# hydradarpa/kalman-hydra

Measured on AMD Instinct MI355X. Metric: frames/sec (Brox flow + EKF update) at 1024^2, higher is better.
Workload: dtype f32 (flow, renders) / f64 (EKF sums and state)

## Files before the change

kalman-hydra_amd/csrc/chol_flow_kernels.h:

```cpp
#pragma once
#include <hip/hip_runtime.h>
#include "dense_kernels.h"

#define FLOW_NT 256
#ifdef HM_STAMP
#define HM_CHAIN_STAMP(c, k) do { if (g_stamp && (threadIdx.x & 63) == 0) g_stamp[(size_t)(4096 + (c)) * 8 + (k)] = clock64(); } while (0)
#else
#define HM_CHAIN_STAMP(c, k) do { } while (0)
#endif
#define FLOW_SENTINEL 0x7FF8DEADBEEF0001ull
#define FLOW_POLL_LIMIT 4000000

struct FlowArgs {
    const double *A;
    double *L;
    double *Lt;
    double *Tinv;
    double *P;
    int n, nrows, nb, nbr;
    unsigned *ctl;
    int stall;
};

__device__ __forceinline__ unsigned long long flow_ld_bits(const double *p)
// ... 346 lines not shown
    double acc = 0.0;
    for (int j = threadIdx.x; j < n; j += 256) {
        const double h = H[(size_t)row * n + j];
        A[(size_t)row * n + j] = invW0[(size_t)row * n + j] + h;
        acc += h * (X0[j] + -1.0 * X[j]);
    }
    for (int o = 32; o > 0; o >>= 1) acc += __shfl_down(acc, o, 64);
    if ((threadIdx.x & 63) == 0) s[threadIdx.x >> 6] = acc;
    __syncthreads();
    if (threadIdx.x == 0) A[(size_t)rhs_row * n + row] = Hz[row] - (((s[0] + s[1]) + s[2]) + s[3]);
}

struct PrepArgs {
    const double *out;
    int N, vsplit, esplit;
    double eZ, eJ, eM, d;
    const int *nb_off, *nb_u, *nb_e;
    const double *invW0, *X0, *X;
    double *A, *Hz, *Hzc;
    int n, rhs_row;
    FlowArgs f;
};

__device__ __forceinline__ double d_job_sum(const double *__restrict__ out, int job, int parts, int idx)
{
    const double *src = out + (size_t)job * MEAS_VSPLIT_MAX * MEAS_OUT;
    double v = src[idx];
    for (int q = 1; q < parts; q++) v += src[q * MEAS_OUT + idx];
    return v;
}

#define PREP_MAX_ENTRIES (4 * (EKF_MAX_STAR + 2))
__global__ __launch_bounds__(256) void k_solve_prep(PrepArgs p)
{
    __shared__ double s_term[PREP_MAX_ENTRIES];
    __shared__ double s_hz;
    const int row = blockIdx.x, t = threadIdx.x, n = p.n;
    if (row >= (int)gridDim.x - FLOW_FILL_WGS) {
        flow_fill_blocks(p.f, (row - ((int)gridDim.x - FLOW_FILL_WGS)) * 256 + t, 256 * FLOW_FILL_WGS);
        return;
    }
    flow_fill_row(p.f, row, t, 256);
    if (row >= n) {
        if (row != p.rhs_row)
            for (int j = t; j < n; j += 256) p.A[(size_t)row * n + j] = 0.0;
        return;
    }
    double *Arow = p.A + (size_t)row * n;
    const double *Wrow = p.invW0 + (size_t)row * n;
    {
        double w[4];
#pragma unroll
        for (int q = 0; q < 4; q++) w[q] = (t + 256 * q < n) ? Wrow[t + 256 * q] : 0.0;
#pragma unroll
        for (int q = 0; q < 4; q++)
            if (t + 256 * q < n) Arow[t + 256 * q] = w[q];
        for (int j = t + 1024; j < n; j += 256) Arow[j] = Wrow[j];
    }
    const int N = p.N, n2 = 2 * N;
    const int v = (row % n2) >> 1, ca = (row & 1) + (row >= n2 ? 2 : 0);
    const int deg = p.nb_off[v + 1] - p.nb_off[v];
    const int entries = min(PREP_MAX_ENTRIES, 4 * (deg + 1));
    double val = 0.0;
    int col = 0;
    if (t < entries) {
        const int q = t >> 2, cb = t & 3;
        int idx = -1, job, parts, u;
        bool weighted;
        if (q == 0) {
            u = v; job = v; parts = p.vsplit;
            const int lo = min(ca, cb), hi = max(ca, cb);
            const int tab[4][4] = {{A_XX, A_XY, A_XVX, A_XVY}, {-1, A_YY, A_YVX, A_YVY}, {-1, -1, A_VXVX, -1}, {-1, -1, -1, A_VYVY}};
            idx = tab[lo][hi];
            weighted = hi < 2;
        } else {
            u = p.nb_u[p.nb_off[v] + q - 1];
            job = N + p.nb_e[p.nb_off[v] + q - 1]; parts = p.esplit;
            const int c1 = v < u ? ca : cb, c2 = v < u ? cb : ca;
            const int tab[4][4] = {{B_XX, B_XY, B_XVX, B_XVY}, {B_YX, B_YY, B_YVX, B_YVY}, {B_VXX, B_VXY, B_VXVX, -1},
                                   {B_VYX, B_VYY, -1, B_VYVY}};
            idx = tab[c1][c2];
            weighted = c1 < 2 && c2 < 2;
        }
        col = 2 * u + (cb & 1) + (cb >= 2 ? n2 : 0);
        if (idx >= 0) {
            const double raw = d_job_sum(p.out, job, parts, idx);
            val = (weighted ? raw : raw / p.eJ) / p.d / p.d;
        }
        s_term[t] = val * (p.X0[col] + -1.0 * p.X[col]);
    } else if (t == 255) {
        double c[4] = {0.0, 0.0, 0.0, 0.0};
        if (ca < 2) {
            const int b0 = ca == 0 ? A_X : A_Y;
            c[0] = d_job_sum(p.out, v, p.vsplit, b0) / p.eZ; c[1] = d_job_sum(p.out, v, p.vsplit, b0 + 1) / p.eJ;
            c[2] = -d_job_sum(p.out, v, p.vsplit, b0 + 2) / p.eJ; c[3] = d_job_sum(p.out, v, p.vsplit, b0 + 3) / p.eM;
        } else if (ca == 2) {
            c[1] = d_job_sum(p.out, v, p.vsplit, A_VX) / p.eJ;
        } else {
            c[2] = -d_job_sum(p.out, v, p.vsplit, A_VY) / p.eJ;
        }
        const double hz = (((c[0] + c[1]) + c[2]) + c[3]) / p.d / 2;
        p.Hz[row] = hz;
        for (int ch = 0; ch < 4; ch++) p.Hzc[(size_t)row * 4 + ch] = c[ch] / p.d / 2;
        s_hz = hz;
    }
    __syncthreads();
    if (t < entries) Arow[col] = Wrow[col] + val;
    if (t == 0) {
        double acc = 0.0;
        for (int i = 0; i < entries; i++) acc += s_term[i];
        p.A[(size_t)p.rhs_row * n + row] = s_hz - acc;
    }
}
```

kalman-hydra_amd/csrc/ekf.hip:

```cpp
#include "hm_common.h"
#include "ekf_kernels.h"
#include "dense_kernels.h"
#include "chol_flow_kernels.h"
#include "project_kernels.h"
#include "predict_kernels.h"
#include "view_kernels.h"
#include "body_kernels.h"
#include "roi_kernels.h"
#include "smooth_kernels.h"
#include <algorithm>
#include <atomic>
#include <chrono>
#include <cmath>
#include <condition_variable>
#include <cstring>
#include <functional>
#include <mutex>
#include <set>
#include <thread>
#include <utility>
#include <vector>

struct Helper {
    std::thread th;
// ... 38 lines not shown
    }
    void stop()
    {
        {
            std::unique_lock<std::mutex> lk(m);
            cv.wait(lk, [&] { return !busy; });
            quit = true;
            cv.notify_all();
        }
        if (th.joinable()) th.join();
    }
};

struct hm_ctx {
    int device, W, H, N, T, E, njobs;
    HmOwner own{1};
    Helper helper;
    bool helper_used = false;
    int tail_async = 1;
    double eps_Z, eps_J, eps_M;
    hipStream_t stream;
    int *d_tri, *d_star_off, *d_star_tri, *d_edges;
    int *d_nb_off = nullptr, *d_nb_u = nullptr, *d_nb_e = nullptr;
    float *d_uv;
    uint8_t *d_tex;
    std::vector<int> edges;
    uint8_t *d_yim, *d_ym;
    float *d_yfx, *d_yfy, *d_yfxm, *d_yfym;
    bool obs_owned = true;
    const uint8_t *o_yim, *o_ym;
    const float *o_yfx, *o_yfy;
    bool have_tex, have_obs, have_ref;
    Targets ref, P, Q;
    TriSetup *d_setup, *d_cfgs;
    int4 *d_ubox;
    int *d_tlist = nullptr, *d_tcount = nullptr;
    unsigned *d_tmask = nullptr;
    double *d_X, *d_out, *d_partial;
    uint8_t *d_im8, *d_m8;
    std::vector<double> X0;
    double *d_HTH;
    double *d_H, *d_Hz, *d_Hzc, *d_invW0, *d_Af[2], *d_T[2], *d_step, *d_Wtmp, *d_X0, *d_Xn, *d_Wprior, *d_gain, *d_Awork, *d_Lt[2];
    std::vector<double> upd_X0;
    int upd_last = -1, upd_prev = -1;
    double *d_Wres;
    double *pin;
// ... 322 lines not shown
    step(upload(h->own, &h->d_star_off, off.data(), off.size()));
    step(upload(h->own, &h->d_star_tri, flat.data(), flat.size()));
    step(upload(h->own, &h->d_edges, h->edges.data(), h->edges.size()));
    {
        std::vector<std::vector<std::pair<int, int>>> nb(N);
        for (int e = 0; e < h->E; e++) {
            const int a = h->edges[2 * e], b = h->edges[2 * e + 1];
            nb[a].push_back(std::make_pair(b, e));
            nb[b].push_back(std::make_pair(a, e));
        }
        std::vector<int> noff(N + 1, 0), nu, ne;
        for (int v = 0; v < N; v++) {
            std::sort(nb[v].begin(), nb[v].end());
            noff[v + 1] = noff[v] + (int)nb[v].size();
            for (const auto &q : nb[v]) { nu.push_back(q.first); ne.push_back(q.second); }
            if (rc == HM_OK && 4 * ((int)nb[v].size() + 1) > PREP_MAX_ENTRIES) {
                hm_set_error("hm_ctx_create: vertex %d has %d neighbours, limit %d", v, (int)nb[v].size(), PREP_MAX_ENTRIES / 4 - 1);
                rc = HM_ERR_ARG;
            }
        }
        step(upload(h->own, &h->d_nb_off, noff.data(), noff.size()));
        step(upload(h->own, &h->d_nb_u, nu.data(), nu.size()));
        step(upload(h->own, &h->d_nb_e, ne.data(), ne.size()));
    }
    hipError_t e = hipSuccess;
    auto dev = [&](auto **p, size_t bytes) { if (e == hipSuccess) e = h->own.alloc(p, bytes); };
    if (rc == HM_OK) {
        const char *pe = getenv("HYDRA_MI_EKF_PRIORITY");
        e = h->own.stream(&h->stream, !(pe && atoi(pe) == 0));
        dev(&h->d_tex, n);
        dev(&h->d_yim, n);
        dev(&h->d_ym, n);
        dev(&h->d_yfx, n * sizeof(float));
        dev(&h->d_yfy, n * sizeof(float));
        dev(&h->d_yfxm, n * sizeof(float));
        dev(&h->d_yfym, n * sizeof(float));
        dev(&h->d_setup, (size_t)T * sizeof(TriSetup));
        dev(&h->d_cfgs, (size_t)N * MEAS_NCFG * (EKF_MAX_STAR + 1) * sizeof(TriSetup));
        dev(&h->d_ubox, (size_t)N * UBOX_STRIDE * sizeof(int4));
        dev(&h->d_tmask, (size_t)N * TMASK_STRIDE * sizeof(unsigned));
        dev(&h->d_tlist, (size_t)N * TMASK_STRIDE * sizeof(int));
        dev(&h->d_tcount, (size_t)N * sizeof(int));
        dev(&h->d_X, (size_t)4 * N * sizeof(double));
        dev(&h->d_out, (size_t)h->njobs * MEAS_VSPLIT_MAX * MEAS_OUT * sizeof(double));
        dev(&h->d_partial, (size_t)h->red_blocks * 4 * sizeof(double));
        h->ntiles = hm_cdiv(W, RI_W) * hm_cdiv(H, 8);
        dev(&h->d_tpart, (size_t)h->ntiles * RI_NV * sizeof(double));
        dev(&h->d_im8, n);
        dev(&h->d_m8, n);
        const size_t n4 = (size_t)4 * N, nn = n4 * n4 * sizeof(double);
        dev(&h->d_H, nn);
        dev(&h->d_HTH, nn);
        if (e == hipSuccess) e = hipMemsetAsync(h->d_HTH, 0, nn, h->stream);
        dev(&h->d_invW0, nn);
        const size_t nn_aug = (size_t)(hm_cdiv((int)n4, DNB) * DNB + DNB) * n4 * sizeof(double);
        dev(&h->d_Af[0], nn_aug);
        dev(&h->d_Af[1], nn_aug);
        dev(&h->d_Awork, nn_aug);
        const size_t ld_bytes = (size_t)hm_cdiv((int)n4, DNB) * DNB * DNB * sizeof(double);
        dev(&h->d_T[0], nn);
        dev(&h->d_T[1], nn);
        dev(&h->d_step, n4 * sizeof(double));
        dev(&h->d_Lt[0], ld_bytes);
        dev(&h->d_Lt[1], ld_bytes);
        dev(&h->d_Wtmp, nn);
        dev(&h->d_flowP, 3 * ld_bytes);
        dev(&h->d_flowctl, 4 * sizeof(unsigned));
        if (e == hipSuccess) e = hipMemsetAsync(h->d_flowctl, 0, 4 * sizeof(unsigned), h->stream);
        dev(&h->d_Hz, n4 * sizeof(double));
        dev(&h->d_Hzc, n4 * 4 * sizeof(double));
        dev(&h->d_Wprior, nn);
        dev(&h->d_gain, n4 * 3 * sizeof(double));
        h->pin_n = 2 * (n4 + RES_HEAD + n4 * 4 + n4 * 3) + 2;
        if (e == hipSuccess) e = h->own.host_alloc(&h->pin, h->pin_n * sizeof(double), hipHostMallocCoherent);
        if (e == hipSuccess) memset(h->pin, 0, h->pin_n * sizeof(double));
        h->pin_scratch = (int *)(h->pin + h->pin_n - 2);
        h->resv.assign(n4 + RES_HEAD, 0.0);
        h->tailv.assign(n4 * 7, 0.0);
        dev(&h->d_X0, n4 * sizeof(double));
        dev(&h->pool.hdr, (size_t)4 * N * sizeof(int));
        dev(&h->pool.overflow, sizeof(int));
        dev(&h->d_area, (size_t)N * sizeof(int));
        h->pool.area = h->d_area;
        if (e == hipSuccess) e = pool_alloc(h, (long long)8 * W * H);
        dev(&h->d_Xn, n4 * sizeof(double));
        for (Targets *t : {&h->ref, &h->P, &h->Q})
            if (e == hipSuccess) e = alloc_targets(h->own, *t, n);
    }
    if (e != hipSuccess) {
        hm_set_error("hm_ctx_create: device allocation failed: %s", hipGetErrorString(e));
        step(HM_ERR_HIP);
// ... 33 lines not shown
        HM_ARG(value >= 2 && value <= 2048, "hm_ctx_tune: chol_flow_wgs must be in 2..2048 (the chain workgroup and at least one task workgroup)");
        h->flow_wgs = value;
    } else if (!strcmp(key, "render_rows")) {
        HM_ARG(value == 8 || value == 16, "hm_ctx_tune: render_rows must be 8 or 16");
        h->render_rows = value;
    } else if (!strcmp(key, "chol_flow_stall")) {
        HM_ARG(value >= 0 && value <= 100000, "hm_ctx_tune: chol_flow_stall must be in 0..100000");
        h->flow_stall = value;
    } else if (!strcmp(key, "result_delay")) {
        HM_ARG(value >= 0 && value <= 5000, "hm_ctx_tune: result_delay must be in 0..5000 (microseconds)");
        h->result_delay = value;
    } else if (!strcmp(key, "tail_async")) {
        HM_ARG(value == 0 || value == 1, "hm_ctx_tune: tail_async must be 0 or 1");
        h->tail_async = value;
    } else if (!strcmp(key, "tail_split")) {
        HM_ARG(value == 0 || value == 1, "hm_ctx_tune: tail_split must be 0 or 1");
        h->tail_split = value;
    } else if (!strcmp(key, "newton_fail")) {
        HM_ARG(value == 0 || value == 1, "hm_ctx_tune: newton_fail must be 0 or 1");
        h->newton_fail = value;
    } else if (!strcmp(key, "speculate")) {
        HM_ARG(value == 0 || value == 1, "hm_ctx_tune: speculate must be 0 or 1");
        h->speculate = value;
    } else if (!strcmp(key, "edge_split")) {
        HM_ARG(value >= 1 && value <= MEAS_VSPLIT_MAX, "hm_ctx_tune: edge_split must be in 1..%d", MEAS_VSPLIT_MAX);
        h->esplit = value;
    } else if (!strcmp(key, "body_stats_cap")) {
        HM_ARG(value >= 1 && value <= BODY_STATS_CAP, "hm_ctx_tune: body_stats_cap must be in 1..%d", BODY_STATS_CAP);
        h->stats_cap = value;
    } else if (!strcmp(key, "body_rec_chunk")) {
        HM_ARG(value >= 0, "hm_ctx_tune: body_rec_chunk must be >= 0 (0: the default size)");
        h->rec_chunk = value;
    } else {
        hm_set_error("hm_ctx_tune: unknown key '%s'", key);
        return HM_ERR_ARG;
    }
    return HM_OK;
}
extern "C" void *hm_ctx_stream(hm_ctx_t h)
{
    (void)ctx_join(h);
    return h ? (void *)h->stream : nullptr;
}
extern "C" int hm_ctx_sync(hm_ctx_t h)
{
    HM_ARG(h != nullptr, "hm_ctx_sync: NULL handle");
// ... 394 lines not shown

extern "C" int hm_error(hm_ctx_t h, const double *X, int masked, double err[4], float *fx, float *fy)
{
    HM_ARG(h && X && err, "hm_error: NULL argument");
    HM_JOIN(h);
    NEED_TEX(h, "hm_error");
    NEED_OBS(h, "hm_error");
    HM_HIP(hipSetDevice(h->device));
    HM_HIP(hipMemcpyAsync(h->d_X, X, (size_t)4 * h->N * sizeof(double), hipMemcpyHostToDevice, h->stream));
    int rc = render_iter(h, h->d_X, h->P, true, masked, false, 2.0);
    if (rc) return rc;
    const int n = h->W * h->H;
    if (fx) HM_HIP(hipMemcpyAsync(fx, h->P.fx, (size_t)n * sizeof(float), hipMemcpyDeviceToHost, h->stream));
    if (fy) HM_HIP(hipMemcpyAsync(fy, h->P.fy, (size_t)n * sizeof(float), hipMemcpyDeviceToHost, h->stream));
    HM_HIP(hipMemcpyAsync(h->h_tpart.data(), h->d_tpart, (size_t)render_strips(h) * RI_NV * sizeof(double), hipMemcpyDeviceToHost, h->stream));
    HM_HIP(stream_wait(h->stream));
    double s6[RI_NV];
    hm_tile_partial_sums(h->h_tpart.data(), render_strips(h), s6);
    for (int k = 0; k < 4; k++) err[k] = s6[k];
    return HM_OK;
}

static int measure_dev(hm_ctx *h, const double *dX, bool ref_ready, double deltaX, int masked, bool regions_ready = false,
                       bool scatter = true)
{
    if (!ref_ready) {
        int rc = render_iter(h, dX, h->ref, false, masked, !regions_ready, deltaX);
        if (rc) return rc;
        regions_ready = true;
    }
    MeasureArgs a;
    measure_args(h, dX, deltaX, masked, a);
    if (!regions_ready) hipLaunchKernelGGL(k_star_regions, dim3(h->N), dim3(REGION_NT), 0, h->stream, a, h->d_area);
    hipLaunchKernelGGL(k_measure_vertex, dim3(h->N, h->vsplit), dim3(MEAS_NT), 0, h->stream, a,
                       (const TriSetup *)h->d_cfgs, (const int4 *)h->d_ubox, (const unsigned *)h->d_tmask);
    if (h->E > 0) hipLaunchKernelGGL(k_measure_edge, dim3(h->E, h->esplit), dim3(MEAS_NT), 0, h->stream, a);
    if (scatter) {
        ScatterArgs s = {h->d_out, h->d_edges, h->N, h->E, h->vsplit, h->esplit, h->eps_Z, h->eps_J, h->eps_M, deltaX, h->d_HTH, h->d_Hz, h->d_Hzc};
        hipLaunchKernelGGL(k_hth_scatter, dim3(hm_cdiv(h->njobs, 4)), dim3(256), 0, h->stream, s);
    }
    HM_HIP(hipGetLastError());
    return HM_OK;
}

static void measure_args(hm_ctx *h, const double *dX, double deltaX, int masked, MeasureArgs &a)
{
    a.m = Mesh{h->W, h->H, h->N, h->T, h->d_tri, h->d_uv, h->d_tex};
    a.topo = StarTopo{h->d_star_off, h->d_star_tri, h->d_edges, h->E};
    a.ref = h->ref;
    a.obs = obs_of(h, masked);
    a.X = dX;
    a.delta = deltaX;
    a.out = h->d_out;
    a.pool = h->pool;
    a.vsplit = h->vsplit;
    a.esplit = h->esplit;
    a.iZ = 1.0 / h->eps_Z; a.iJ = 1.0 / h->eps_J; a.iM = 1.0 / h->eps_M;
    a.cfgs = h->d_cfgs;
    a.ubox = h->d_ubox;
// ... 57 lines not shown
    if (!first_done) hipLaunchKernelGGL(k_chol_first, dim3(1), dim3(64), 0, st, A, Lt, n);
    for (int k = 0; k < nb; k++) {
        const int mr = nbr - k - 1, mc = std::max(nb - k - 1, 1);
        hipLaunchKernelGGL(k_chol_step, dim3((mc + k + 1) * (mr + 1)), dim3(256), 0, st, A, L, Lt, T, M, n, nrows, nb, k, mc, mc + k + 1, mr + 1);
    }
}

static void chol_inverse(hm_ctx *h, int n, const double *T, double *out, hipStream_t st = nullptr)
{
    const int nb = hm_cdiv(n, DNB);
    hipLaunchKernelGGL(k_ttt, dim3(nb, nb), dim3(256), 0, st ? st : h->stream, T, n, out);
}

static int flow_status(hm_ctx *h, const char *who)
{
    if (!h->chol_flow) return HM_OK;
    unsigned ctl[2] = {0, 0};
    HM_HIP(hipMemcpyAsync(ctl, h->d_flowctl, sizeof ctl, hipMemcpyDeviceToHost, h->stream));
    HM_HIP(hipStreamSynchronize(h->stream));
    if (ctl[1]) { hm_set_error("%s: the factorisation launch gave up waiting for a block (chol_flow time-out)", who); return HM_ERR_HIP; }
    return HM_OK;
}

static double *solve_step(hm_ctx *h, int slot, double deltaX)
{
    const int n4 = 4 * h->N;
    double *A = h->d_Awork;
    const int rhs_index = hm_cdiv(n4, DNB) * DNB;
    double *rhs_row = A + (size_t)rhs_index * n4;
    {
        const int nb = hm_cdiv(n4, DNB), nrows = aug_rows(n4);
        PrepArgs p;
        p.out = h->d_out; p.N = h->N; p.vsplit = h->vsplit; p.esplit = h->esplit;
        p.eZ = h->eps_Z; p.eJ = h->eps_J; p.eM = h->eps_M; p.d = deltaX;
        p.nb_off = h->d_nb_off; p.nb_u = h->d_nb_u; p.nb_e = h->d_nb_e;
        p.invW0 = h->d_invW0; p.X0 = h->d_X0; p.X = h->d_X;
        p.A = A; p.Hz = h->d_Hz; p.Hzc = h->d_Hzc; p.n = n4; p.rhs_row = rhs_index;
        p.f = FlowArgs{A, h->d_Af[slot], h->d_Lt[slot], h->d_T[slot], h->d_flowP, n4, nrows, nb, hm_cdiv(nrows, DNB), h->d_flowctl, 0};
        hipLaunchKernelGGL(k_solve_prep, dim3(nrows + FLOW_FILL_WGS), dim3(256), 0, h->stream, p);
    }
    if (h->d_Wres == h->d_Wtmp) h->d_Wres = nullptr;
    chol_factor(h, A, h->d_Af[slot], h->d_Lt[slot], h->d_T[slot], h->d_Wtmp, n4, true, h->chol_flow != 0);
    const double *yrow = h->d_Af[slot] + (rhs_row - A);
    hipLaunchKernelGGL(k_tvec, dim3(hm_cdiv(n4, TV_COLS)), dim3(TV_COLS * TV_ROWS), 0, h->stream, h->d_T[slot], n4, yrow, h->d_step, h->d_X0,
                       h->d_Xn);
    return h->d_step;
}

static int prior_inverse(hm_ctx *h, const double *W_prior, hipStream_t st = nullptr)
{
    if (!st) st = h->stream;
    const int n4 = 4 * h->N;
    const size_t nnb = (size_t)n4 * n4 * sizeof(double);
    if (W_prior)
        HM_HIP(hipMemcpyAsync(h->d_Wprior, W_prior, nnb, hipMemcpyHostToDevice, st));
    else if (h->d_Wres != h->d_Wprior)
        HM_HIP(hipMemcpyAsync(h->d_Wprior, h->d_Wres, nnb, hipMemcpyDeviceToDevice, st));
    if (!h->chol_flow) HM_HIP(hipMemcpyAsync(h->d_Awork, h->d_Wprior, nnb, hipMemcpyDeviceToDevice, st));
    h->d_Wres = h->d_Wprior;
    HM_HIP(hipMemsetAsync(h->d_flowctl, 0, 4 * sizeof(unsigned), st));
    chol_factor(h, h->chol_flow ? h->d_Wprior : h->d_Awork, h->d_Af[0], h->d_Lt[0], h->d_Wtmp, h->d_invW0, n4, false, false, st);
    chol_inverse(h, n4, h->d_Wtmp, h->d_invW0, st);
// ... 318 lines not shown
    auto chain_collect = [&]() -> int {
        int r = hb_wait(h->stream3, h->pin_n4 + n4, 0, (size_t)n4 + 2, hb_stamp(h->n4_ticket), h->n4v.data(), "hm_update_run (state prediction)");
        h->n4_pending = false;
        if (r) return r;
        r = hb_wait(h->stream3, h->pin_pm + n4, 0, (size_t)n4 + 1, hb_stamp(h->pm_ticket), h->pmv.data(), "hm_update_run (projectmask)");
        if (r) return r;
        h->chain_pred.assign(h->n4v.begin(), h->n4v.begin() + n4);
        h->chain_proj.assign(h->pmv.begin(), h->pmv.begin() + n4);
        h->chain_its = (int)h->n4v[n4];
        h->chain_moved = (int)h->pmv[n4];
        if (h->n4v[n4 + 1] != 0.0) return 2;
        X0 = h->chain_proj; Xcur = X0; Xold = X0;
        h->upd_X0 = X0;
        h->X0 = X0;
        return HM_OK;
    };
    bool collected = !chained;
    if (!chained) HM_HIP(hipMemcpyAsync(h->d_X, h->d_X0, (size_t)n4 * sizeof(double), hipMemcpyDeviceToDevice, h->stream));
    double *const pin_res = h->pin, *const pin_tail = h->pin + 2 * ((size_t)n4 + RES_HEAD);
    const double *const res = h->resv.data();
    int niter = 0, accepted = 0;
    bool reverted = false, conv = false, ref_ready = false, regions_ahead = false, grown = false;
    double eold = 0.0;
    bool spec = false;
    auto unspec = [&]() {
        if (spec) { std::swap(h->ref, h->P); std::swap(h->d_X, h->d_Xn); spec = false; }
    };
    for (int it = 0; it < max_iter; it++) {
        if (!spec) {
            rc = measure_dev(h, h->d_X, ref_ready, deltaX, masked, regions_ahead, false);
            if (rc) return rc;
        }
        spec = false;
        if (next_mask && it == 0) {
            HM_HIP(h->own.event(&h->ev_m0));
            HM_HIP(hipEventRecord(h->ev_m0, h->stream));
        }
        if (collected) h->X0 = Xcur;
        h->have_ref = true;
        const int slot = h->upd_last == 0 ? 1 : 0;
        rc = ctx_join(h);
        if (rc) return rc;
        double *rhs_row = solve_step(h, slot, deltaX);
        regions_ahead = it + 1 < max_iter;
        rc = render_iter(h, h->d_Xn, h->P, true, masked, regions_ahead, deltaX);
        if (rc) return rc;
        hipLaunchKernelGGL(k_iter_result, dim3(1), dim3(256), 0, h->stream, rhs_row, n4, h->d_tpart,
                           render_strips(h), h->pool.overflow, (const unsigned *)h->d_flowctl, pin_res, (double)(++h->run_ticket),
                           h->result_delay);
        HM_HIP(hipGetLastError());
        if (h->speculate && regions_ahead) {
            std::swap(h->ref, h->P);
            std::swap(h->d_X, h->d_Xn);
            spec = true;
            rc = measure_dev(h, h->d_X, true, deltaX, masked, true, false);
            if (rc) { unspec(); return rc; }
        }
        const auto dbg_t0 = std::chrono::steady_clock::now();
        if (next_mask && it == 0) {
            rc = ensure_stream2(h);
            if (rc == HM_OK) { HM_HIP(hipStreamWaitEvent(h->stream2, h->ev_m0, 0)); rc = prepare_mask(h, next_mask); }
            if (rc) { unspec(); return rc; }
            next_mask = nullptr;
        }
        if (!collected) {
            rc = chain_collect();
            if (rc) { unspec(); (void)hipStreamSynchronize(h->stream); return rc; }
            collected = true;
        }
        rc = hb_wait(h->stream, pin_res, 0, (size_t)n4 + RES_HEAD, hb_stamp(h->run_ticket), h->resv.data(), "hm_update_run");
        if (rc) { unspec(); return rc; }
        if (getenv("HYDRA_MI_TRACE")) {
            const double ms = std::chrono::duration<double, std::milli>(std::chrono::steady_clock::now() - dbg_t0).count();
            if (ms > 1.5) fprintf(stderr, "[hydra_mi] hm_update_run: iteration %d waited %.2f ms for its result\n", it, ms);
        }
        if (res[n4 + 4] != 0.0) {
            unspec();
            if (grown) { hm_set_error("hm_update_run: the star regions do not fit the difference-image pool"); return HM_ERR_STATE; }
// ... 1624 lines not shown
```

kalman-hydra_amd/csrc/ekf_kernels.h:

```cpp
#pragma once
#include <hip/hip_runtime.h>
#include <stdint.h>

#define EKF_SUB 256
#define EKF_MAX_STAR 24
#define EKF_TILE 16
#define EKF_MAX_TRI 4096

struct TriSetup {
    double ea[3], eb[3], ec[3];
    double ecb[3];
    int cmin, cmax, rmin, rmax;
    int tl[3];
    float inv;
    int i0, i1, i2;
    float ux[3], uy[3], ax[3], ay[3];
};

__device__ __forceinline__ void d_tri_attr(TriSetup &s, const float *__restrict__ uv, const double *__restrict__ X, int N)
{
    const int id[3] = {s.i0, s.i1, s.i2};
    for (int k = 0; k < 3; k++) {
        s.ux[k] = uv[2 * id[k]];
        s.uy[k] = uv[2 * id[k] + 1];
// ... 191 lines not shown
    const int p = r * m.W + c;
    if (MODE != 2) { out.acc[p] = acc; out.fx[p] = fx; out.fy[p] = fy; out.cnt[p] = cnt; }
    if (MODE != 0) ids[p] = 256 * min(sg, 255) + min(sb, 255);
}

__global__ void k_resolve(Targets t, uint8_t *__restrict__ im, uint8_t *__restrict__ mk, int n)
{
    int p = blockIdx.x * blockDim.x + threadIdx.x;
    if (p >= n) return;
    if (im) im[p] = (uint8_t)(t.acc[p] > 255 ? 255 : t.acc[p]);
    if (mk) mk[p] = t.cnt[p] > 0 ? 255 : 0;
}

__global__ void k_mask_flow(const uint8_t *__restrict__ ym, const float *__restrict__ fx, const float *__restrict__ fy,
                            float *__restrict__ fxm, float *__restrict__ fym, int n)
{
    int p = blockIdx.x * blockDim.x + threadIdx.x;
    if (p >= n) return;
    float mm = (float)ym[p];
    fxm[p] = mm * fx[p];
    fym[p] = mm * fy[p];
}

template <int NACC, int NT>
__device__ inline void d_block_reduce(double (&a)[NACC], double *s_red , double *out)
{
#pragma unroll
    for (int k = 0; k < NACC; k++) {
        double v = a[k];
#pragma unroll
        for (int o = 32; o > 0; o >>= 1) v += __shfl_down(v, o, 64);
        a[k] = v;
    }
    const int lane = threadIdx.x & 63, wv = threadIdx.x >> 6;
    if (lane == 0)
        for (int k = 0; k < NACC; k++) s_red[wv * NACC + k] = a[k];
    __syncthreads();
    if (threadIdx.x < NACC) {
        double v = 0.0;
        for (int w = 0; w < NT / 64; w++) v += s_red[w * NACC + threadIdx.x];
        out[threadIdx.x] = v;
    }
}

struct Obs {
    const uint8_t *yim;
    const float *yfx, *yfy;
    const uint8_t *ym;
};

#define RED_NT 256
__global__ __launch_bounds__(RED_NT) void k_jz(Targets ref, Targets p, Obs o, int n, double *__restrict__ partial)
{
    __shared__ double s_red[(RED_NT / 64) * 4];
    double a[4] = {0, 0, 0, 0};
    for (int i = blockIdx.x * RED_NT + threadIdx.x; i < n; i += gridDim.x * RED_NT) {
        int rim = ref.acc[i] > 255 ? 255 : ref.acc[i], pim = p.acc[i] > 255 ? 255 : p.acc[i];
        int rm = ref.cnt[i] > 0 ? 255 : 0, pm = p.cnt[i] > 0 ? 255 : 0;
        double z = ((double)o.yim[i] - (double)rim) / 255.0;
        double zm = (255.0 * (double)o.ym[i] - (double)rm) / 255.0;
        float zfx = o.yfx[i] - ref.fx[i];
        float zfy = o.yfy[i] + ref.fy[i];
        a[0] += ((double)(pim - rim) / 255.0) * z;
        a[1] += (double)(p.fx[i] - ref.fx[i]) * (double)zfx;
// ... 524 lines not shown
            a.pool.xfx[pp] = dxp.fx; a.pool.xfy[pp] = dxp.fy; a.pool.yfx[pp] = dyp.fx; a.pool.yfy[pp] = dyp.fy;
            a.pool.vxfx[pp] = dvxp.fx; a.pool.vyfy[pp] = dvyp.fy;
        }
    }
    if (park && listed >= 0)
        for (int t = blockIdx.y * MEAS_NT + threadIdx.x; t < ntiles; t += MEAS_NT * gridDim.y)
            if (tmask[(size_t)v * a.tmask_stride + t] == 0) a.pool.live[base / 64 + t] = 0;
    d_block_reduce<A_NV, MEAS_NT>(acc, s_red, a.out + ((size_t)job * MEAS_VSPLIT_MAX + blockIdx.y) * MEAS_OUT);
}

struct EdgeTile {
    short2 ax, ay, bx, by;
    float axfx, axfy, ayfx, ayfy, avx, avy, bxfx, bxfy, byfx, byfy, bvx, bvy;
};
__device__ __forceinline__ EdgeTile d_edge_load(const DPool &P, long long pv, long long pw)
{
    EdgeTile t;
    t.ax = P.xi[pv]; t.bx = P.xi[pw]; t.ay = P.yi[pv]; t.by = P.yi[pw];
    t.axfx = P.xfx[pv]; t.axfy = P.xfy[pv]; t.ayfx = P.yfx[pv]; t.ayfy = P.yfy[pv]; t.avx = P.vxfx[pv]; t.avy = P.vyfy[pv];
    t.bxfx = P.xfx[pw]; t.bxfy = P.xfy[pw]; t.byfx = P.yfx[pw]; t.byfy = P.yfy[pw]; t.bvx = P.vxfx[pw]; t.bvy = P.vyfy[pw];
    return t;
}

__global__ __launch_bounds__(MEAS_NT) void k_measure_edge(MeasureArgs a)
{
    __shared__ double s_red[(MEAS_NT / 64) * MEAS_OUT];
    __shared__ double s_k255[511];
    const double *k255 = s_k255 + 255;
    d_fill_k255(s_k255, MEAS_NT);
    __syncthreads();
    const int N = a.m.N;
    const int e = blockIdx.x;
    const int v = a.topo.edges[2 * e], w = a.topo.edges[2 * e + 1];
    const int *hv = a.pool.hdr + 4 * v, *hw = a.pool.hdr + 4 * w;
    const int tx0 = max(hv[0], hw[0]) >> 3, ty0 = max(hv[1], hw[1]) >> 3;
    const int tx1 = min(hv[0] + hv[2], hw[0] + hw[2]) >> 3, ty1 = min(hv[1] + hv[3], hw[1] + hw[3]) >> 3;
    const int ntx = tx1 - tx0, nty = ty1 - ty0;
    const int vx0 = hv[0] >> 3, vy0 = hv[1] >> 3, vnx = hv[2] >> 3;
    const int wx0 = hw[0] >> 3, wy0 = hw[1] >> 3, wnx = hw[2] >> 3;
    __shared__ long long s_sum[(MEAS_NT / 64) * 3];
    long long bv, bw, total;
    d_region_sums<MEAS_NT>(a.pool.area, N, v, w, bv, bw, total, s_sum);
    const int nt = (total <= a.pool.cap && ntx > 0 && nty > 0) ? ntx * nty : 0;
    double acc[B_NV];
#pragma unroll
    for (int k = 0; k < B_NV; k++) acc[k] = 0.0;
    const DPool &P = a.pool;
    const int lane = threadIdx.x & 63;
    const int gw = blockIdx.y * (MEAS_NT / 64) + (threadIdx.x >> 6), nwaves = (MEAS_NT / 64) * gridDim.y;
    const double iZ = a.iZ, iJ = a.iJ, iM = a.iM;
    const int ntxd = ntx > 0 ? ntx : 1;
    for (int first = 0; first < nt; first += 64 * nwaves) {
        const int cand = first + lane * nwaves + gw;
        int tv = 0, tw = 0;
        bool go = false;
        if (cand < nt) {
            const int tx = tx0 + cand % ntxd, ty = ty0 + cand / ntxd;
            tv = (ty - vy0) * vnx + (tx - vx0);
            tw = (ty - wy0) * wnx + (tx - wx0);
            go = (P.live[bv / 64 + tv] != 0) & (P.live[bw / 64 + tw] != 0);
        }
        unsigned long long todo = __ballot(go);
        if (todo == 0) continue;
        int l = __builtin_ctzll(todo);
        todo &= todo - 1;
        EdgeTile nx = d_edge_load(P, bv + (long long)__shfl(tv, l, 64) * 64 + lane, bw + (long long)__shfl(tw, l, 64) * 64 + lane);
        for (;;) {
            const EdgeTile t = nx;
            const bool more = todo != 0;
            if (more) {
                l = __builtin_ctzll(todo);
                todo &= todo - 1;
// ... 3 lines not shown
                const double axim = k255[t.ax.x], axm = k255[t.ax.y];
                const double ayim = k255[t.ay.x], aym = k255[t.ay.y];
                const double bxim = k255[t.bx.x], bxm = k255[t.bx.y];
                const double byim = k255[t.by.x], bym = k255[t.by.y];
                const double axfx = t.axfx, axfy = t.axfy, ayfx = t.ayfx, ayfy = t.ayfy;
                const double bxfx = t.bxfx, bxfy = t.bxfy, byfx = t.byfx, byfy = t.byfy;
                const double avx = t.avx, avy = t.avy, bvx = t.bvx, bvy = t.bvy;
                const double wxi = axim * iZ, wxf = axfx * iJ, wxg = axfy * iJ, wxm = axm * iM;
                const double wyi = ayim * iZ, wyf = ayfx * iJ, wyg = ayfy * iJ, wym = aym * iM;
                acc[B_XX] = fma(wxm, bxm, fma(wxg, bxfy, fma(wxf, bxfx, fma(wxi, bxim, acc[B_XX]))));
                acc[B_XY] = fma(wxm, bym, fma(wxg, byfy, fma(wxf, byfx, fma(wxi, byim, acc[B_XY]))));
                acc[B_YX] = fma(wym, bxm, fma(wyg, bxfy, fma(wyf, bxfx, fma(wyi, bxim, acc[B_YX]))));
                acc[B_YY] = fma(wym, bym, fma(wyg, byfy, fma(wyf, byfx, fma(wyi, byim, acc[B_YY]))));
                acc[B_XVX] = fma(axfx, bvx, acc[B_XVX]); acc[B_YVX] = fma(ayfx, bvx, acc[B_YVX]);
                acc[B_VXX] = fma(avx, bxfx, acc[B_VXX]); acc[B_VXY] = fma(avx, byfx, acc[B_VXY]);
                acc[B_VXVX] = fma(avx, bvx, acc[B_VXVX]);
                acc[B_XVY] = fma(axfy, bvy, acc[B_XVY]); acc[B_YVY] = fma(ayfy, bvy, acc[B_YVY]);
                acc[B_VYX] = fma(avy, bxfy, acc[B_VYX]); acc[B_VYY] = fma(avy, byfy, acc[B_VYY]);
                acc[B_VYVY] = fma(avy, bvy, acc[B_VYVY]);
            }
            if (!more) break;
        }
    }
    d_block_reduce<B_NV, MEAS_NT>(acc, s_red, a.out + ((size_t)(N + e) * MEAS_VSPLIT_MAX + blockIdx.y) * MEAS_OUT);
}

#define RI_CHUNK 32
#define RI_GROUPS 256
#define RI_W 64
#define RI_H 16
struct IterRenderArgs {
    Mesh m;
    const double *X;
    Targets out;
    Obs o;
    const float *raw_fx, *raw_fy;
    double *partial;
    int tiles_x, tiles_y, with_err, n_regions;
};
#define RI_NV 6
struct RenderShared {
    unsigned mask[EKF_MAX_TRI / 32];
    TriSetup cand[RI_CHUNK];
    double red[(256 / 64) * RI_NV];
    unsigned band[RI_W / 8];
};

// ... 273 lines not shown
```

Measured before the change: 336.9.

## Fuse edge measurement with solve prep via per-vertex arrival counters

Merges k_measure_edge and k_solve_prep into one launch. Each edge block stores its partial sums with agent-scope atomics, then bumps an arrival counter for both endpoint vertices. The last block to arrive for a vertex builds that vertex's four A rows, one wave per row. Pad rows, isolated vertices and flow-fill blocks get their own dedicated blocks. This removes a kernel boundary and lets row prep overlap edge measurement, but adds atomics, fences, and serial row-prep work in the tail blocks.

```diff
diff --git a/kalman-hydra_amd/csrc/chol_flow_kernels.h b/kalman-hydra_amd/csrc/chol_flow_kernels.h
--- a/kalman-hydra_amd/csrc/chol_flow_kernels.h
+++ b/kalman-hydra_amd/csrc/chol_flow_kernels.h
@@ -392,7 +392,7 @@
     FlowArgs f;
 };
 
-__device__ __forceinline__ double d_job_sum(const double *__restrict__ out, int job, int parts, int idx)
+__device__ __forceinline__ double d_job_sum(const double *out, int job, int parts, int idx)
 {
     const double *src = out + (size_t)job * MEAS_VSPLIT_MAX * MEAS_OUT;
     double v = src[idx];
@@ -401,40 +401,35 @@
 }
 
 #define PREP_MAX_ENTRIES (4 * (EKF_MAX_STAR + 2))
-__global__ __launch_bounds__(256) void k_solve_prep(PrepArgs p)
-{
-    __shared__ double s_term[PREP_MAX_ENTRIES];
-    __shared__ double s_hz;
-    const int row = blockIdx.x, t = threadIdx.x, n = p.n;
-    if (row >= (int)gridDim.x - FLOW_FILL_WGS) {
-        flow_fill_blocks(p.f, (row - ((int)gridDim.x - FLOW_FILL_WGS)) * 256 + t, 256 * FLOW_FILL_WGS);
-        return;
-    }
-    flow_fill_row(p.f, row, t, 256);
-    if (row >= n) {
-        if (row != p.rhs_row)
-            for (int j = t; j < n; j += 256) p.A[(size_t)row * n + j] = 0.0;
-        return;
-    }
+struct PrepRowShared {
+    double term[PREP_MAX_ENTRIES], val[PREP_MAX_ENTRIES];
+    int col[PREP_MAX_ENTRIES];
+    double hz;
+};
+
+template <int NT>
+__device__ __forceinline__ void d_prep_row(const PrepArgs &p, int row, int t, PrepRowShared &s)
+{
+    const int n = p.n;
     double *Arow = p.A + (size_t)row * n;
     const double *Wrow = p.invW0 + (size_t)row * n;
     {
-        double w[4];
-#pragma unroll
-        for (int q = 0; q < 4; q++) w[q] = (t + 256 * q < n) ? Wrow[t + 256 * q] : 0.0;
-#pragma unroll
-        for (int q = 0; q < 4; q++)
-            if (t + 256 * q < n) Arow[t + 256 * q] = w[q];
-        for (int j = t + 1024; j < n; j += 256) Arow[j] = Wrow[j];
+        constexpr int Q = NT >= 256 ? 4 : 16;
+        for (int j0 = 0; j0 < n; j0 += Q * NT) {
+            double w[Q];
+#pragma unroll
+            for (int q = 0; q < Q; q++) w[q] = (j0 + t + NT * q < n) ? Wrow[j0 + t + NT * q] : 0.0;
+#pragma unroll
+            for (int q = 0; q < Q; q++)
+                if (j0 + t + NT * q < n) Arow[j0 + t + NT * q] = w[q];
+        }
     }
     const int N = p.N, n2 = 2 * N;
     const int v = (row % n2) >> 1, ca = (row & 1) + (row >= n2 ? 2 : 0);
     const int deg = p.nb_off[v + 1] - p.nb_off[v];
     const int entries = min(PREP_MAX_ENTRIES, 4 * (deg + 1));
-    double val = 0.0;
-    int col = 0;
-    if (t < entries) {
-        const int q = t >> 2, cb = t & 3;
+    for (int i = t; i < entries; i += NT) {
+        const int q = i >> 2, cb = i & 3;
         int idx = -1, job, parts, u;
         bool weighted;
         if (q == 0) {
@@ -452,13 +447,17 @@
             idx = tab[c1][c2];
             weighted = c1 < 2 && c2 < 2;
         }
-        col = 2 * u + (cb & 1) + (cb >= 2 ? n2 : 0);
+        const int col = 2 * u + (cb & 1) + (cb >= 2 ? n2 : 0);
+        double val = 0.0;
         if (idx >= 0) {
             const double raw = d_job_sum(p.out, job, parts, idx);
             val = (weighted ? raw : raw / p.eJ) / p.d / p.d;
         }
-        s_term[t] = val * (p.X0[col] + -1.0 * p.X[col]);
-    } else if (t == 255) {
+        s.val[i] = val;
+        s.col[i] = col;
+        s.term[i] = val * (p.X0[col] + -1.0 * p.X[col]);
+    }
+    if (t == NT - 1) {
         double c[4] = {0.0, 0.0, 0.0, 0.0};
         if (ca < 2) {
             const int b0 = ca == 0 ? A_X : A_Y;
@@ -472,13 +471,96 @@
         const double hz = (((c[0] + c[1]) + c[2]) + c[3]) / p.d / 2;
         p.Hz[row] = hz;
         for (int ch = 0; ch < 4; ch++) p.Hzc[(size_t)row * 4 + ch] = c[ch] / p.d / 2;
-        s_hz = hz;
+        s.hz = hz;
     }
     __syncthreads();
-    if (t < entries) Arow[col] = Wrow[col] + val;
+    for (int i = t; i < entries; i += NT) Arow[s.col[i]] = Wrow[s.col[i]] + s.val[i];
     if (t == 0) {
         double acc = 0.0;
-        for (int i = 0; i < entries; i++) acc += s_term[i];
-        p.A[(size_t)p.rhs_row * n + row] = s_hz - acc;
-    }
-}
+        for (int i = 0; i < entries; i++) acc += s.term[i];
+        p.A[(size_t)p.rhs_row * n + row] = s.hz - acc;
+    }
+}
+
+__device__ __forceinline__ void d_prep_pad_row(const PrepArgs &p, int row, int t, int nt)
+{
+    flow_fill_row(p.f, row, t, nt);
+    if (row != p.rhs_row)
+        for (int j = t; j < p.n; j += nt) p.A[(size_t)row * p.n + j] = 0.0;
+}
+
+__global__ __launch_bounds__(256) void k_solve_prep(PrepArgs p)
+{
+    __shared__ PrepRowShared s;
+    const int row = blockIdx.x, t = threadIdx.x;
+    if (row >= (int)gridDim.x - FLOW_FILL_WGS) {
+        flow_fill_blocks(p.f, (row - ((int)gridDim.x - FLOW_FILL_WGS)) * 256 + t, 256 * FLOW_FILL_WGS);
+        return;
+    }
+    if (row >= p.n) {
+        d_prep_pad_row(p, row, t, 256);
+        return;
+    }
+    flow_fill_row(p.f, row, t, 256);
+    d_prep_row<256>(p, row, t, s);
+}
+
+struct EdgePrepArgs {
+    unsigned *arrive;
+    const int *iso;
+    int n_iso, E;
+};
+
+__device__ __forceinline__ void d_prep_vertex_rows(const PrepArgs &p, int v, PrepRowShared *s )
+{
+    const int wv = threadIdx.x >> 6, lane = threadIdx.x & 63;
+    const int row = 2 * v + (wv & 1) + (wv >= 2 ? 2 * p.N : 0);
+    flow_fill_row(p.f, row, lane, 64);
+    d_prep_row<64>(p, row, lane, s[wv]);
+}
+
+__global__ __launch_bounds__(MEAS_NT) void k_measure_edge_prep(MeasureArgs a, PrepArgs p, EdgePrepArgs x)
+{
+    static_assert(MEAS_NT == 256, "one wave per row of a vertex");
+    __shared__ double s_red[(MEAS_NT / 64) * MEAS_OUT];
+    __shared__ double s_k255[511];
+    __shared__ long long s_sum[(MEAS_NT / 64) * 3];
+    __shared__ PrepRowShared s_row[4];
+    __shared__ int s_done[2];
+    const int t = threadIdx.x;
+    const int npad = p.f.nrows - p.n;
+    int b = blockIdx.x;
+    if (b < npad) { d_prep_pad_row(p, p.n + b, t, MEAS_NT); return; }
+    b -= npad;
+    if (b < x.n_iso) { d_prep_vertex_rows(p, x.iso[b], s_row); return; }
+    b -= x.n_iso;
+    if (b < FLOW_FILL_WGS) { flow_fill_blocks(p.f, b * MEAS_NT + t, MEAS_NT * FLOW_FILL_WGS); return; }
+    b -= FLOW_FILL_WGS;
+    const int e = b % x.E, part = b / x.E;
+    d_measure_edge<true>(a, e, part, a.esplit, s_red, s_k255, s_sum);
+    asm volatile("s_waitcnt vmcnt(0)" ::: "memory");
+    __syncthreads();
+    if (t == 0) {
+        bool any = false;
+        for (int k = 0; k < 2; k++) {
+            const int u = a.topo.edges[2 * e + k];
+            const unsigned want = (unsigned)(p.nb_off[u + 1] - p.nb_off[u]) * (unsigned)a.esplit;
+            const unsigned had = __hip_atomic_fetch_add(x.arrive + u, 1u, __ATOMIC_RELAXED, __HIP_MEMORY_SCOPE_AGENT);
+            const bool last = had + 1 == want;
+            if (last) __hip_atomic_store(x.arrive + u, 0u, __ATOMIC_RELAXED, __HIP_MEMORY_SCOPE_AGENT);
+            s_done[k] = last ? u : -1;
+            any = any || last;
+        }
+        if (any) {
+            __builtin_amdgcn_fence(__ATOMIC_ACQUIRE, "agent");
+            asm volatile("s_waitcnt vmcnt(0)" ::: "memory");
+        }
+    }
+    __syncthreads();
+    for (int k = 0; k < 2; k++) {
+        const int u = s_done[k];
+        if (u < 0) continue;
+        d_prep_vertex_rows(p, u, s_row);
+        __syncthreads();
+    }
+}
diff --git a/kalman-hydra_amd/csrc/ekf.hip b/kalman-hydra_amd/csrc/ekf.hip
--- a/kalman-hydra_amd/csrc/ekf.hip
+++ b/kalman-hydra_amd/csrc/ekf.hip
@@ -84,6 +84,10 @@
     hipStream_t stream;
     int *d_tri, *d_star_off, *d_star_tri, *d_edges;
     int *d_nb_off = nullptr, *d_nb_u = nullptr, *d_nb_e = nullptr;
+    unsigned *d_arrive = nullptr;
+    int *d_iso = nullptr;
+    int n_iso = 0;
+    int prep_fused = 1;
     float *d_uv;
     uint8_t *d_tex;
     std::vector<int> edges;
@@ -452,6 +456,12 @@
         step(upload(h->own, &h->d_nb_off, noff.data(), noff.size()));
         step(upload(h->own, &h->d_nb_u, nu.data(), nu.size()));
         step(upload(h->own, &h->d_nb_e, ne.data(), ne.size()));
+        std::vector<int> iso;
+        for (int v = 0; v < N; v++)
+            if (nb[v].empty()) iso.push_back(v);
+        h->n_iso = (int)iso.size();
+        iso.push_back(-1);
+        step(upload(h->own, &h->d_iso, iso.data(), iso.size()));
     }
     hipError_t e = hipSuccess;
     auto dev = [&](auto **p, size_t bytes) { if (e == hipSuccess) e = h->own.alloc(p, bytes); };
@@ -497,6 +507,8 @@
         dev(&h->d_flowP, 3 * ld_bytes);
         dev(&h->d_flowctl, 4 * sizeof(unsigned));
         if (e == hipSuccess) e = hipMemsetAsync(h->d_flowctl, 0, 4 * sizeof(unsigned), h->stream);
+        dev(&h->d_arrive, (size_t)N * sizeof(unsigned));
+        if (e == hipSuccess) e = hipMemsetAsync(h->d_arrive, 0, (size_t)N * sizeof(unsigned), h->stream);
         dev(&h->d_Hz, n4 * sizeof(double));
         dev(&h->d_Hzc, n4 * 4 * sizeof(double));
         dev(&h->d_Wprior, nn);
@@ -576,6 +588,9 @@
     } else if (!strcmp(key, "speculate")) {
         HM_ARG(value == 0 || value == 1, "hm_ctx_tune: speculate must be 0 or 1");
         h->speculate = value;
+    } else if (!strcmp(key, "prep_fused")) {
+        HM_ARG(value == 0 || value == 1, "hm_ctx_tune: prep_fused must be 0 (k_measure_edge, k_solve_prep) or 1 (one launch)");
+        h->prep_fused = value;
     } else if (!strcmp(key, "edge_split")) {
         HM_ARG(value >= 1 && value <= MEAS_VSPLIT_MAX, "hm_ctx_tune: edge_split must be in 1..%d", MEAS_VSPLIT_MAX);
         h->esplit = value;
@@ -1016,7 +1031,7 @@
 }
 
 static int measure_dev(hm_ctx *h, const double *dX, bool ref_ready, double deltaX, int masked, bool regions_ready = false,
-                       bool scatter = true)
+                       bool scatter = true, bool edges = true)
 {
     if (!ref_ready) {
         int rc = render_iter(h, dX, h->ref, false, masked, !regions_ready, deltaX);
@@ -1028,7 +1043,7 @@
     if (!regions_ready) hipLaunchKernelGGL(k_star_regions, dim3(h->N), dim3(REGION_NT), 0, h->stream, a, h->d_area);
     hipLaunchKernelGGL(k_measure_vertex, dim3(h->N, h->vsplit), dim3(MEAS_NT), 0, h->stream, a,
                        (const TriSetup *)h->d_cfgs, (const int4 *)h->d_ubox, (const unsigned *)h->d_tmask);
-    if (h->E > 0) hipLaunchKernelGGL(k_measure_edge, dim3(h->E, h->esplit), dim3(MEAS_NT), 0, h->stream, a);
+    if (h->E > 0 && edges) hipLaunchKernelGGL(k_measure_edge, dim3(h->E, h->esplit), dim3(MEAS_NT), 0, h->stream, a);
     if (scatter) {
         ScatterArgs s = {h->d_out, h->d_edges, h->N, h->E, h->vsplit, h->esplit, h->eps_Z, h->eps_J, h->eps_M, deltaX, h->d_HTH, h->d_Hz, h->d_Hzc};
         hipLaunchKernelGGL(k_hth_scatter, dim3(hm_cdiv(h->njobs, 4)), dim3(256), 0, h->stream, s);
@@ -1132,22 +1147,39 @@
     return HM_OK;
 }
 
-static double *solve_step(hm_ctx *h, int slot, double deltaX)
+static PrepArgs prep_args(hm_ctx *h, int slot, double deltaX)
+{
+    const int n4 = 4 * h->N, nb = hm_cdiv(n4, DNB), nrows = aug_rows(n4);
+    double *A = h->d_Awork;
+    PrepArgs p;
+    p.out = h->d_out; p.N = h->N; p.vsplit = h->vsplit; p.esplit = h->esplit;
+    p.eZ = h->eps_Z; p.eJ = h->eps_J; p.eM = h->eps_M; p.d = deltaX;
+    p.nb_off = h->d_nb_off; p.nb_u = h->d_nb_u; p.nb_e = h->d_nb_e;
+    p.invW0 = h->d_invW0; p.X0 = h->d_X0; p.X = h->d_X;
+    p.A = A; p.Hz = h->d_Hz; p.Hzc = h->d_Hzc; p.n = n4; p.rhs_row = nb * DNB;
+    p.f = FlowArgs{A, h->d_Af[slot], h->d_Lt[slot], h->d_T[slot], h->d_flowP, n4, nrows, nb, hm_cdiv(nrows, DNB), h->d_flowctl, 0};
+    return p;
+}
+
+static void edge_prep(hm_ctx *h, int slot, double deltaX, int masked)
+{
+    MeasureArgs a;
+    measure_args(h, h->d_X, deltaX, masked, a);
+    const PrepArgs p = prep_args(h, slot, deltaX);
+    const EdgePrepArgs x = {h->d_arrive, h->d_iso, h->n_iso, h->E};
+    const int extra = (p.f.nrows - p.n) + h->n_iso + FLOW_FILL_WGS;
+    hipLaunchKernelGGL(k_measure_edge_prep, dim3(extra + h->E * h->esplit), dim3(MEAS_NT), 0, h->stream, a, p, x);
+}
+
+static double *solve_step(hm_ctx *h, int slot, double deltaX, bool prepped = false)
 {
     const int n4 = 4 * h->N;
     double *A = h->d_Awork;
     const int rhs_index = hm_cdiv(n4, DNB) * DNB;
     double *rhs_row = A + (size_t)rhs_index * n4;
-    {
-        const int nb = hm_cdiv(n4, DNB), nrows = aug_rows(n4);
-        PrepArgs p;
-        p.out = h->d_out; p.N = h->N; p.vsplit = h->vsplit; p.esplit = h->esplit;
-        p.eZ = h->eps_Z; p.eJ = h->eps_J; p.eM = h->eps_M; p.d = deltaX;
-        p.nb_off = h->d_nb_off; p.nb_u = h->d_nb_u; p.nb_e = h->d_nb_e;
-        p.invW0 = h->d_invW0; p.X0 = h->d_X0; p.X = h->d_X;
-        p.A = A; p.Hz = h->d_Hz; p.Hzc = h->d_Hzc; p.n = n4; p.rhs_row = rhs_index;
-        p.f = FlowArgs{A, h->d_Af[slot], h->d_Lt[slot], h->d_T[slot], h->d_flowP, n4, nrows, nb, hm_cdiv(nrows, DNB), h->d_flowctl, 0};
-        hipLaunchKernelGGL(k_solve_prep, dim3(nrows + FLOW_FILL_WGS), dim3(256), 0, h->stream, p);
+    if (!prepped) {
+        const PrepArgs p = prep_args(h, slot, deltaX);
+        hipLaunchKernelGGL(k_solve_prep, dim3(p.f.nrows + FLOW_FILL_WGS), dim3(256), 0, h->stream, p);
     }
     if (h->d_Wres == h->d_Wtmp) h->d_Wres = nullptr;
     chol_factor(h, A, h->d_Af[slot], h->d_Lt[slot], h->d_T[slot], h->d_Wtmp, n4, true, h->chol_flow != 0);
@@ -1512,17 +1544,18 @@
     int niter = 0, accepted = 0;
     bool reverted = false, conv = false, ref_ready = false, regions_ahead = false, grown = false;
     double eold = 0.0;
+    const bool fused = h->prep_fused != 0;
     bool spec = false;
     auto unspec = [&]() {
         if (spec) { std::swap(h->ref, h->P); std::swap(h->d_X, h->d_Xn); spec = false; }
     };
     for (int it = 0; it < max_iter; it++) {
         if (!spec) {
-            rc = measure_dev(h, h->d_X, ref_ready, deltaX, masked, regions_ahead, false);
+            rc = measure_dev(h, h->d_X, ref_ready, deltaX, masked, regions_ahead, false, !fused);
             if (rc) return rc;
         }
         spec = false;
-        if (next_mask && it == 0) {
+        if (next_mask && it == 0 && !fused) {
             HM_HIP(h->own.event(&h->ev_m0));
             HM_HIP(hipEventRecord(h->ev_m0, h->stream));
         }
@@ -1531,7 +1564,14 @@
         const int slot = h->upd_last == 0 ? 1 : 0;
         rc = ctx_join(h);
         if (rc) return rc;
-        double *rhs_row = solve_step(h, slot, deltaX);
+        if (fused) {
+            edge_prep(h, slot, deltaX, masked);
+            if (next_mask && it == 0) {
+                HM_HIP(h->own.event(&h->ev_m0));
+                HM_HIP(hipEventRecord(h->ev_m0, h->stream));
+            }
+        }
+        double *rhs_row = solve_step(h, slot, deltaX, fused);
         regions_ahead = it + 1 < max_iter;
         rc = render_iter(h, h->d_Xn, h->P, true, masked, regions_ahead, deltaX);
         if (rc) return rc;
@@ -1543,7 +1583,7 @@
             std::swap(h->ref, h->P);
             std::swap(h->d_X, h->d_Xn);
             spec = true;
-            rc = measure_dev(h, h->d_X, true, deltaX, masked, true, false);
+            rc = measure_dev(h, h->d_X, true, deltaX, masked, true, false, !fused);
             if (rc) { unspec(); return rc; }
         }
         const auto dbg_t0 = std::chrono::steady_clock::now();
diff --git a/kalman-hydra_amd/csrc/ekf_kernels.h b/kalman-hydra_amd/csrc/ekf_kernels.h
--- a/kalman-hydra_amd/csrc/ekf_kernels.h
+++ b/kalman-hydra_amd/csrc/ekf_kernels.h
@@ -237,7 +237,7 @@
     fym[p] = mm * fy[p];
 }
 
-template <int NACC, int NT>
+template <int NACC, int NT, bool WT = false>
 __device__ inline void d_block_reduce(double (&a)[NACC], double *s_red , double *out)
 {
 #pragma unroll
@@ -254,7 +254,9 @@
     if (threadIdx.x < NACC) {
         double v = 0.0;
         for (int w = 0; w < NT / 64; w++) v += s_red[w * NACC + threadIdx.x];
-        out[threadIdx.x] = v;
+        if (WT) __hip_atomic_store((unsigned long long *)(out + threadIdx.x), (unsigned long long)__double_as_longlong(v),
+                                   __ATOMIC_RELAXED, __HIP_MEMORY_SCOPE_AGENT);
+        else out[threadIdx.x] = v;
     }
 }
 
@@ -825,15 +827,14 @@
     return t;
 }
 
-__global__ __launch_bounds__(MEAS_NT) void k_measure_edge(MeasureArgs a)
-{
-    __shared__ double s_red[(MEAS_NT / 64) * MEAS_OUT];
-    __shared__ double s_k255[511];
+template <bool WT>
+__device__ __forceinline__ void d_measure_edge(const MeasureArgs &a, int e, int part, int parts, double *s_red, double *s_k255,
+                                               long long *s_sum)
+{
     const double *k255 = s_k255 + 255;
     d_fill_k255(s_k255, MEAS_NT);
     __syncthreads();
     const int N = a.m.N;
-    const int e = blockIdx.x;
     const int v = a.topo.edges[2 * e], w = a.topo.edges[2 * e + 1];
     const int *hv = a.pool.hdr + 4 * v, *hw = a.pool.hdr + 4 * w;
     const int tx0 = max(hv[0], hw[0]) >> 3, ty0 = max(hv[1], hw[1]) >> 3;
@@ -841,7 +842,6 @@
     const int ntx = tx1 - tx0, nty = ty1 - ty0;
     const int vx0 = hv[0] >> 3, vy0 = hv[1] >> 3, vnx = hv[2] >> 3;
     const int wx0 = hw[0] >> 3, wy0 = hw[1] >> 3, wnx = hw[2] >> 3;
-    __shared__ long long s_sum[(MEAS_NT / 64) * 3];
     long long bv, bw, total;
     d_region_sums<MEAS_NT>(a.pool.area, N, v, w, bv, bw, total, s_sum);
     const int nt = (total <= a.pool.cap && ntx > 0 && nty > 0) ? ntx * nty : 0;
@@ -850,7 +850,7 @@
     for (int k = 0; k < B_NV; k++) acc[k] = 0.0;
     const DPool &P = a.pool;
     const int lane = threadIdx.x & 63;
-    const int gw = blockIdx.y * (MEAS_NT / 64) + (threadIdx.x >> 6), nwaves = (MEAS_NT / 64) * gridDim.y;
+    const int gw = part * (MEAS_NT / 64) + (threadIdx.x >> 6), nwaves = (MEAS_NT / 64) * parts;
     const double iZ = a.iZ, iJ = a.iJ, iM = a.iM;
     const int ntxd = ntx > 0 ? ntx : 1;
     for (int first = 0; first < nt; first += 64 * nwaves) {
@@ -900,7 +900,15 @@
             if (!more) break;
         }
     }
-    d_block_reduce<B_NV, MEAS_NT>(acc, s_red, a.out + ((size_t)(N + e) * MEAS_VSPLIT_MAX + blockIdx.y) * MEAS_OUT);
+    d_block_reduce<B_NV, MEAS_NT, WT>(acc, s_red, a.out + ((size_t)(N + e) * MEAS_VSPLIT_MAX + part) * MEAS_OUT);
+}
+
+__global__ __launch_bounds__(MEAS_NT) void k_measure_edge(MeasureArgs a)
+{
+    __shared__ double s_red[(MEAS_NT / 64) * MEAS_OUT];
+    __shared__ double s_k255[511];
+    __shared__ long long s_sum[(MEAS_NT / 64) * 3];
+    d_measure_edge<false>(a, blockIdx.x, blockIdx.y, gridDim.y, s_red, s_k255, s_sum);
 }
 
 #define RI_CHUNK 32
```

After: 327.4. -2.8%, worse.
